# semicolonTransistor/rust-ray-tracing

Hardware: AMD Instinct MI355X
Metric: Msamples/s (pixels×spp/s), 1920×1080·512spp·500 spheres; 1/2/4/8 GPU (higher is better)
Workload: dtype f32

## Files before the change

### rust-ray-tracing_amd/csrc/rt_common.hpp

```cpp
#pragma once
#include <hip/hip_runtime.h>
#include <stdint.h>
#include <stdio.h>
#include <stdlib.h>
#include <string.h>
#include <algorithm>
#include <array>
#include <initializer_list>
#include <chrono>
#include <cmath>
#include <limits>
#include <mutex>
#include <string>
#include <type_traits>
#include <vector>

#include "../../include/rt_mi355x.h"
#include "rt_device.hpp"
#include "rt_formats.hpp"
#include "rt_experiments.hpp"

namespace rt {

template <typename T> struct alignas(64) SphGroup { T v[64 / sizeof(T)]; };

template <typename T>
__device__ __forceinline__ SphGroup<T> load_group(const __attribute__((address_space(4))) T* f, uint32_t g) {
    constexpr int NE = 64 / sizeof(T);
    SphGroup<T> r;
#pragma unroll
    for (int e = 0; e < NE; ++e) r.v[e] = f[g * NE + e];
    return r;
}

typedef float f2 __attribute__((ext_vector_type(2)));
struct Q4 { uint32_t x, y, z, w; };

struct alignas(32) BoxGroup { float v[kBoxFloats]; };
__device__ __forceinline__ BoxGroup load_box(const __attribute__((address_space(4))) float* f, uint32_t g) {
    BoxGroup r;
#pragma unroll
    for (uint32_t e = 0; e < kBoxFloats; ++e) r.v[e] = f[g * kBoxFloats + e];
    return r;
}
__device__ __forceinline__ f2 fma2(f2 a, f2 b, f2 c) { return __builtin_elementwise_fma(a, b, c); }

template <typename T> struct KParams {
    const T* sph;
    const T* cen;
    uint32_t n_groups;
    const MatT<T>* mats;
    uint32_t n_spheres;
    uint32_t W, H;
    double rW, rH;
    T center[3], ulc[3], vu[3], vv[3], du[3], dv[3];
    uint32_t spp, P, C, depth, flags, s_sel, k0, k1;
    uint32_t row_begin, row_step, col_begin, col_count;
    uint8_t* rgb;
    double* lin;
    unsigned long long* segs;
    uint32_t* err;
    uint32_t* counter;
    uint32_t blk_g;
    uint32_t n_items;
    char* scratch;
    size_t scratch_stride;
    uint32_t vbytes, sbytes;
    uint32_t swide;
    const T* camsph;
    const float* fsph;
    const float* camf;
    uint32_t n_fgroups;
    float f_cmax, f_r2max;
    float f_r2min;
    float f_ir2, f_hir2, f_isr;
    const float* cull;
    const float* cullc;
    uint32_t n_clp, n_supc;
    const T* camx;
    const T* rsph;
    const float* rfsph;
    const float* ftop;
    const float* fsup;
    const float* fmeg;
    uint32_t n_mg;
    const float* lfsph;
    const float* lclb;
    const float* lsup;
    const float* lmeg;
    const float* lgig;
    uint32_t n_gg;
    float l_r2max, l_hir2, l_isr;
    const uint64_t* mtiers;
    float mt_lo[3], mt_inv;
    uint32_t mt_n[3];
    const uint32_t* ridx;
    uint32_t n_top, n_xg, n_xs;
};

template <typename T> struct SParams {
    KParams<T> k;
    char* rec;
    uint32_t S, nsub;
    uint32_t n_pix;
};

template <typename T> struct WParams {
    SParams<T> s;
    uint32_t s_begin, s_base;
    uint32_t P_cap;
};

struct MapItem { uint32_t pixel, first, end, pad; };
template <typename T> struct IParams {
    WParams<T> w;
    const MapItem* items;
};
template <typename T> struct LParams {
    WParams<T> w;
    const uint32_t* list;
};

constexpr int kSegShards = 256;
constexpr uint32_t kFlagPinholeInternal = 0x80000000u;
constexpr int kWavesF32 = 6;
constexpr int kWavesF64 = 4;
constexpr int kWavesMegaF32 = 6;
constexpr uint64_t kW6PixelsPerWave = 24;
template <typename T> constexpr int kWavesModes = sizeof(T) == 4 ? 6 : 4;
constexpr int kSegStride = 32;

enum WorkCounter : uint32_t {
    kWBox = 0,
    kWFilt = 1,
    kWExact = 2,
    kWCone = 3,
    kWCExact = 4,
    kNWork = 5,
};
constexpr int kWorkSlot = 11;
constexpr int kDirectSkySlot = 16;
static_assert(kWorkSlot + kNWork <= kDirectSkySlot && kDirectSkySlot < kSegStride, "counters past the shard's slots");
__shared__ unsigned long long g_work[4][kNWork];
__device__ __forceinline__ void work_add(uint32_t i, uint32_t n) {
    const uint32_t first = (uint32_t)__builtin_ctzll(__builtin_amdgcn_read_exec());
    if ((threadIdx.x & 63u) == first) atomicAdd(&g_work[threadIdx.x >> 6][i], (unsigned long long)n);
}


__device__ __forceinline__ uint32_t lanes_below(unsigned long long m) {
    return __builtin_amdgcn_mbcnt_hi((uint32_t)(m >> 32), __builtin_amdgcn_mbcnt_lo((uint32_t)m, 0u));
}

template <typename T> using cptr = const __attribute__((address_space(4))) T*;

template <typename T> __device__ __forceinline__ cptr<KParams<T>> cold_args() {
    cptr<KParams<T>> k = (cptr<KParams<T>>)__builtin_amdgcn_kernarg_segment_ptr();
    asm volatile("" : "+s"(k));
    return k;
}
template <typename T> __device__ __forceinline__ cptr<SParams<T>> cold_split_args() {
    cptr<SParams<T>> k = (cptr<SParams<T>>)__builtin_amdgcn_kernarg_segment_ptr();
    asm volatile("" : "+s"(k));
    return k;
}
template <typename T> __device__ __forceinline__ cptr<WParams<T>> cold_window_args() {
    cptr<WParams<T>> k = (cptr<WParams<T>>)__builtin_amdgcn_kernarg_segment_ptr();
    asm volatile("" : "+s"(k));
    return k;
}
template <typename T> __device__ __forceinline__ cptr<IParams<T>> cold_items_args() {
    cptr<IParams<T>> k = (cptr<IParams<T>>)__builtin_amdgcn_kernarg_segment_ptr();
    asm volatile("" : "+s"(k));
    return k;
}
// ... 90 lines not shown
```

### rust-ray-tracing_amd/csrc/rt_experiments.hpp

```cpp
#pragma once

#if defined(RT_PRODUCT) && defined(RT_EXPERIMENT)
#error "RT_PRODUCT and RT_EXPERIMENT are exclusive"
#endif
#if defined(RT_PRODUCT) && (defined(RT_EXP_BLOCK_SAMPLES) || defined(RT_EXP_TMUL) || defined(RT_EXP_LMAP_CAP) ||      \
                            defined(RT_EXP_DUP_FINISH) || defined(RT_EXP_DUP_CAMRAY) || defined(RT_EXP_DUP_CAM) ||     \
                            defined(RT_EXP_DUP_SCATTER) || defined(RT_EXP_DUP_SWEEP) || defined(RT_EXP_DUP_CLBOX) ||   \
                            defined(RT_EXP_DUP_FILTER) || defined(RT_EXP_DUP_SUPBOX) || defined(RT_EXP_DUP_MEGABOX) || \
                            defined(RT_EXP_DUP_PLIST) || defined(RT_EXP_DUP_REPLAY) || defined(RT_EXP_DUP_REDUCE) ||   \
                            defined(RT_EXP_TIMELINE) || \
                            defined(RT_KSTATS))
#error "an experiment macro in the product build"
#endif
#ifndef RT_SRC_HASH
#define RT_SRC_HASH "unknown"
#endif
#ifdef RT_EXPERIMENT
#define RT_BUILD_KIND "experiment"
#else
#define RT_BUILD_KIND "product"
#endif

namespace rt {

#ifdef RT_EXP_BLOCK_SAMPLES
constexpr uint32_t kBlockSamples = RT_EXP_BLOCK_SAMPLES;
#else
constexpr uint32_t kBlockSamples = 32768;
#endif
#ifdef RT_EXP_TMUL
constexpr uint32_t kTMul = RT_EXP_TMUL;
#else
constexpr uint32_t kTMul = 8;
#endif
#ifdef RT_EXP_LMAP_CAP
constexpr uint32_t kLMapCap = RT_EXP_LMAP_CAP;
#else
constexpr uint32_t kLMapCap = 512;
#endif

#ifdef RT_KSTATS
__shared__ unsigned long long g_kst[4][8];
__device__ __forceinline__ void kstat(uint32_t i, uint32_t n = 1) {
    const unsigned long long ex = __builtin_amdgcn_read_exec();
    if ((threadIdx.x & 63u) == (uint32_t)__builtin_ctzll(ex)) atomicAdd(&g_kst[threadIdx.x >> 6][i], (unsigned long long)n);
}
#define KSTAT(...) kstat(__VA_ARGS__)
#else
#define KSTAT(...) ((void)0)
#endif

}
```

### rust-ray-tracing_amd/csrc/rt_kernel.hip

```cpp
#include "rt_trace.hpp"
#include "rt_layout.hpp"
#include "rt_split_plan.hpp"
#include "rt_progressive_plan.hpp"

#include <chrono>
#include <mutex>
#include <string>

using namespace rt;

static thread_local std::string g_err;
static int fail(int code, const std::string& msg) {
    g_err = msg;
    return code;
}
#define HIPCHK(x)                                                                     \
    do {                                                                              \
        hipError_t e_ = (x);                                                          \
        if (e_ != hipSuccess) return fail(RT_ERR_HIP, std::string(#x ": ") + hipGetErrorString(e_)); \
    } while (0)

struct DeviceBuffer {
    void* p = nullptr;
    size_t bytes = 0;
// ... 51 lines not shown
    PinnedStage& operator=(const PinnedStage&) = delete;
    PinnedStage& operator=(PinnedStage&& o) noexcept {
        if (this != &o) {
            reset();
            p = o.p; bytes = o.bytes; ev = o.ev; pending = o.pending;
            o.p = nullptr; o.bytes = 0; o.ev = nullptr; o.pending = false;
        }
        return *this;
    }
    ~PinnedStage() { reset(); }
    void reset() {
        if (pending) (void)hipEventSynchronize(ev);
        if (ev) (void)hipEventDestroy(ev);
        if (p) (void)hipHostFree(p);
        p = nullptr; bytes = 0; ev = nullptr; pending = false;
    }
};
static int stage_reserve(PinnedStage& g, size_t n) {
    if (!g.ev) HIPCHK(hipEventCreateWithFlags(&g.ev, hipEventDisableTiming));
    if (g.pending) {
        HIPCHK(hipEventSynchronize(g.ev));
        g.pending = false;
    }
    if (n <= g.bytes) return RT_OK;
    if (g.p) HIPCHK(hipHostFree(g.p));
    g.p = nullptr;
    g.bytes = 0;
    HIPCHK(hipHostMalloc(&g.p, n, hipHostMallocDefault));
    g.bytes = n;
    return RT_OK;
}

template <typename T> struct DeviceScene {
    DeviceBuffer sph, cen, fsph, rsph, rfsph, top, sup, meg, lfs, lbx[4], clus, mats;
    DeviceBuffer cam, camf, camx, cull, cullc;
    TableConsts k;
    struct CamKey { bool valid = false; double center[3] = {0, 0, 0}; uint32_t scalar = 0, off = 0; } camkey;
    void reset() { *this = DeviceScene(); }
};
template <typename T> static int upload_scene(DeviceScene<T>& d, const SceneTables<T>& t) {
    int rc = RT_OK;
    auto up = [&](DeviceBuffer& dst, const auto& v) { if (rc == RT_OK) rc = upload(dst, v); };
    auto room = [&](DeviceBuffer& dst, size_t bytes) { if (rc == RT_OK) rc = reserve(dst, bytes); };
    up(d.sph, t.sph); up(d.cen, t.cen); up(d.fsph, t.fsph);
    up(d.rsph, t.rsph); up(d.rfsph, t.rfsph);
    up(d.top, t.top); up(d.sup, t.sup); up(d.meg, t.meg);
    up(d.lfs, t.lfs);
    for (int lv = 0; lv < 4; ++lv) up(d.lbx[lv], t.lbx[lv]);
    up(d.clus, t.clus); up(d.mats, t.mats);
    room(d.cam, t.cam_bytes.cam); room(d.camf, t.cam_bytes.camf); room(d.camx, t.cam_bytes.camx);
    room(d.cull, t.cam_bytes.cull); room(d.cullc, t.cam_bytes.cullc);
    d.k = t.k;
    return rc;
}

struct CountClass {
    uint32_t spp, first, n;
};

struct rt_context {
    int device = 0;
    hipStream_t stream = nullptr;
    hipEvent_t ev_first = nullptr, ev_last = nullptr;
    bool have_first = false;
    DeviceScene<float> d32;
    DeviceScene<double> d64;
    DeviceBuffer ridx, mtiers;
    SceneCounts n;
    template <typename T> DeviceScene<T>& scene() {
        if constexpr (sizeof(T) == 8) return d64; else return d32;
    }
    DeviceBuffer segs, err;
    DeviceBuffer counter;
    DeviceBuffer scratch;
    DeviceBuffer records;
    int n_cu = 0;
    uint64_t samples = 0, pixels = 0;
    hipStream_t last_stream = nullptr;
    bool have_last = false;
// ... 203 lines not shown
    constexpr int W = kWavesSplit<T>;
    return mega ? trace_paths_items<T, W, CAMQ, true> : trace_paths_items<T, W, CAMQ, false>;
}
constexpr uint64_t kScratchBudget = 24ull << 30;

struct FrameArgs {
    const rt_camera* cam;
    uint32_t depth, spp;
    uint64_t seed;
    uint32_t flags;
    rt_tile_range rg;
    void* rgb;
    void* lin;
};
struct SessionWindow {
    char* rec;
    uint32_t cap, s_begin, s_base, S, nsub;
    bool trace, finish;
};

template <typename T>
static void scene_params(rt_context* c, KParams<T>& p) {
    const DeviceScene<T>& d = c->scene<T>();
    const SceneCounts& n = c->n;
    p.sph = (const T*)d.sph.p;
    p.cen = (const T*)d.cen.p;
    p.n_groups = d.k.n_groups;
    p.fsph = (const float*)d.fsph.p;
    p.n_fgroups = n.n_fgroups;
    p.rsph = (const T*)d.rsph.p;
    p.rfsph = (const float*)d.rfsph.p;
    p.ftop = (const float*)d.top.p;
    p.fsup = (const float*)d.sup.p;
    p.fmeg = (const float*)d.meg.p;
    p.n_mg = n.n_mg;
    p.lfsph = (const float*)d.lfs.p;
    p.lclb = (const float*)d.lbx[0].p;
    p.lsup = (const float*)d.lbx[1].p;
    p.lmeg = (const float*)d.lbx[2].p;
    p.lgig = (const float*)d.lbx[3].p;
    p.n_gg = n.n_gg;
    p.mtiers = (const uint64_t*)c->mtiers.p;
    for (int a = 0; a < 3; ++a) { p.mt_lo[a] = n.mt_lo[a]; p.mt_n[a] = n.mt_n[a]; }
    p.mt_inv = n.mt_inv;
    p.l_r2max = d.k.l_r2max;
    p.l_hir2 = d.k.l_hir2;
    p.l_isr = d.k.l_isr;
    p.ridx = (const uint32_t*)c->ridx.p;
    p.n_top = n.n_top;
    p.n_xg = n.n_xg;
    p.n_xs = n.n_xs;
    p.f_cmax = d.k.f_cmax;
    p.f_r2max = d.k.f_r2max;
    p.f_r2min = d.k.f_r2min;
    p.f_ir2 = d.k.f_ir2;
    p.f_hir2 = d.k.f_hir2;
    p.f_isr = d.k.f_isr;
    p.mats = (const MatT<T>*)d.mats.p;
    p.n_spheres = n.n_spheres;
    p.segs = (unsigned long long*)c->segs.p;
    p.err = (uint32_t*)c->err.p;
    p.counter = (uint32_t*)c->counter.p;
}

template <typename T>
static void frame_params(const FrameArgs& a, KParams<T>& p) {
    const rt_camera* cam = a.cam;
// ... 878 lines not shown
                                       uint32_t* items, uint64_t items_capacity) {
    const int rc = progressive_map_plan(n_pixels, done, target, resident_waves, samples_per_item, n_items, items,
                                        items_capacity);
    if (rc != kPlanOk)
        return fail(rc, "rt_progressive_map_plan: a NULL array or output, no pixels, a target below done, too small an "
                        "item capacity (invalid); a target above 2^20, more than 0x7FFFFFFF pixels or items (unsupported)");
    return RT_OK;
}

extern "C" int rt_progressive_end(rt_context* c) {
    if (!c) return fail(RT_ERR_INVALID, "rt_progressive_end: NULL context");
    rt_context::Session& s = c->prog;
    if (!s.open) return fail(RT_ERR_INVALID, "rt_progressive_end: no session open on this context");
    HIPCHK(hipSetDevice(c->device));
    if (s.have_stream) HIPCHK(hipStreamSynchronize(s.stream));
    HIPCHK(hipFree(s.rec));
    s = rt_context::Session{};
    return RT_OK;
}

extern "C" int rt_context_collect(rt_context* c, void* stream, rt_stats* out) {
    if (!c) return fail(RT_ERR_INVALID, "rt_context_collect: NULL context");
    HIPCHK(hipSetDevice(c->device));
    hipStream_t st = (hipStream_t)stream;
    HIPCHK(hipStreamSynchronize(st));
    std::vector<unsigned long long> segs(kSegShards * kSegStride);
    uint32_t err = 0;
    HIPCHK(hipMemcpy(segs.data(), c->segs.p, segs.size() * sizeof(unsigned long long), hipMemcpyDeviceToHost));
    HIPCHK(hipMemcpy(&err, c->err.p, sizeof(uint32_t), hipMemcpyDeviceToHost));
    float ms = 0.f;
    if (c->have_first) HIPCHK(hipEventElapsedTime(&ms, c->ev_first, c->ev_last));
    HIPCHK(hipMemset(c->segs.p, 0, segs.size() * sizeof(unsigned long long)));
    HIPCHK(hipMemset(c->err.p, 0, 16));
    uint64_t total = 0, slots = 0, iters = 0, dsky = 0, kst[8] = {0, 0, 0, 0, 0, 0, 0, 0}, work[kNWork] = {};
    for (int i = 0; i < kSegShards; ++i)
        for (int j = 0; j < 8; ++j) kst[j] += segs[(size_t)i * kSegStride + 3 + j];
    if (kst[0] | kst[1] | kst[2] | kst[3])
        fprintf(stderr, "rt_kstats: general taken_groups %llu sweeps %llu clusters %llu top_groups %llu  camera "
                "candidates %llu sweeps %llu  finish_pixel %llu  filter_lanes_passing %llu\n",
                (unsigned long long)kst[0], (unsigned long long)kst[1], (unsigned long long)kst[4],
                (unsigned long long)kst[5], (unsigned long long)kst[2], (unsigned long long)kst[3],
                (unsigned long long)kst[6], (unsigned long long)kst[7]);
    for (int i = 0; i < kSegShards; ++i) {
        total += segs[(size_t)i * kSegStride];
        slots += segs[(size_t)i * kSegStride + 1];
        iters += segs[(size_t)i * kSegStride + 2];
        dsky += segs[(size_t)i * kSegStride + kDirectSkySlot];
        for (uint32_t j = 0; j < kNWork; ++j) work[j] += segs[(size_t)i * kSegStride + kWorkSlot + j];
    }
    if (out) {
        memset(out, 0, sizeof(*out));
        out->kernel_ms = ms;
        out->pixels = c->pixels;
        out->samples = c->samples;
        out->ray_segments = total;
        out->lane_slots = slots;
        out->bounce_iters = iters;
        out->pixels_per_second = ms > 0.f ? (double)c->pixels / ((double)ms * 1e-3) : 0.0;
        out->box_groups = work[kWBox];
        out->filter_groups = work[kWFilt];
        out->exact_tests = work[kWExact];
        out->cone_tests = work[kWCone];
        out->camera_exact_tests = work[kWCExact];
        out->direct_sky_samples = dsky;
        out->kernel_id = c->last_kernel_id;
        out->kernel_wg_per_cu = c->last_wg_per_cu;
    }
    c->have_first = false;
    c->pixels = c->samples = 0;
    c->last_kernel_id = c->last_wg_per_cu = 0;
    if (err) return fail(RT_ERR_RANGE, "a pixel channel exceeded 2.0 (Color::to_u8_array would panic, color.rs:55-57)");
    return RT_OK;
}

extern "C" int rt_device_alloc(rt_context* c, size_t bytes, void** out) {
// ... 48 lines not shown
```

### rust-ray-tracing_amd/csrc/rt_layout.hpp

```cpp
#pragma once
#include <stdint.h>
#include <string.h>
#include <algorithm>
#include <array>
#include <cmath>
#include <limits>
#include <vector>

#include "../../include/rt_mi355x.h"
#include "rt_formats.hpp"

using namespace rt;

static inline float round_up_f32(double v) {
    float f = (float)v;
    if ((double)f < v) f = std::nextafter(f, std::numeric_limits<float>::infinity());
    return f;
}

template <typename T>
static void pack_scene(const rt_scene* s, std::vector<T>& grp, std::vector<T>& cen, std::vector<MatT<T>>& mats,
                       uint32_t& n_groups) {
    const uint32_t G = kGroup<T>;
    const uint32_t n = s->n_spheres;
// ... 529 lines not shown
                const double dx = (double)cen[4 * i] - C[0], dy = (double)cen[4 * i + 1] - C[1],
                             dz = (double)cen[4 * i + 2] - C[2];
                R = std::max(R, std::sqrt(dx * dx + dy * dy + dz * dz) + std::fabs((double)cen[4 * i + 3]));
            }
        out[4 * at] = C[0]; out[4 * at + 1] = C[1]; out[4 * at + 2] = C[2];
        out[4 * at + 3] = std::isfinite(R) ? R * (1.0 + 0x1.0p-40) : INFINITY;
    };
    for (uint32_t k = 0; k < ncl; ++k) sphere(k, k, 1);
    if (n_supc)
        for (uint32_t k = 0; k < nsup; ++k) sphere(n_clp + k, 4 * k, 4);
}

static std::vector<float> inline_stream(const std::vector<float>& src, size_t n_xg, const std::vector<float>* rg32,
                                        const std::vector<uint32_t>& ridx, const std::vector<float>* frame) {
    const size_t blk = 96, ngf = src.size() / 16 - 1, nxg = n_xg, nk = (ngf - nxg) / 4;
    std::vector<float> rx((size_t)16 * nxg + blk * nk + 32, 0.0f);
    for (size_t g = 0; g < 16 * nxg; ++g) rx[g] = src[g];
    for (size_t k = 0; k < nk; ++k) {
        float* b = &rx[16 * nxg + blk * k];
        for (size_t j = 0; j < 64; ++j) b[j] = src[16 * (nxg + 4 * k) + j];
        for (size_t q = 0; q < 4; ++q) {
            const size_t g = nxg + 4 * k + q;
            uint32_t rec[8] = {0u, 0u, 0u, 0u, 0u, 0u, 0u, 0u};
            if (rg32) for (int h = 0; h < 4; ++h) memcpy(&rec[h], &(*rg32)[16 * g + 8 * (h / 2) + 6 + (h % 2)], 4);
            for (int j = 0; j < 4; ++j) rec[4 + j] = 4 * g + j < ridx.size() ? ridx[4 * g + j] : 0xFFFFFFFFu;
            memcpy(b + 64 + 8 * q, rec, 32);
        }
        if (frame) for (size_t j = 0; j < 4; ++j) { b[64 + j] = (*frame)[8 * k + j]; b[72 + j] = (*frame)[8 * k + 4 + j]; }
    }
    for (size_t j = 0; j < 16; ++j) rx[16 * nxg + blk * nk + j] = src[16 * ngf + j];
    return rx;
}

struct TableConsts {
    uint32_t n_groups = 0;
    float f_cmax = 0, f_r2max = 0, f_r2min = 0;
    float f_ir2 = 0, f_hir2 = 0, f_isr = 0;
    float l_r2max = 0, l_r2min = 0;
    float l_hir2 = 0, l_isr = 0;
};
struct CamTableBytes { size_t cam = 0, camf = 0, camx = 0, cull = 0, cullc = 0; };

template <typename T> struct SceneTables {
    std::vector<T> sph, cen;
    std::vector<float> fsph;
    std::vector<T> rsph;
    std::vector<float> rfsph;
    std::vector<float> top, sup, meg;
    std::vector<float> lfs;
    std::vector<float> lbx[4];
    std::vector<double> clus;
    std::vector<MatT<T>> mats;
    TableConsts k;
    CamTableBytes cam_bytes;
};
struct SceneCounts {
    uint32_t n_spheres = 0;
    uint32_t n_fgroups = 0;
    uint32_t n_top = 0, n_xg = 0, n_xs = 0;
    uint32_t n_mg = 0, n_gg = 0;
    uint32_t n_cslots = 0, n_clp = 0;
    uint32_t n_supc = 0;
    uint32_t n_cull = 0;
    float mt_lo[3] = {0, 0, 0}, mt_inv = 0;
    uint32_t mt_n[3] = {1, 1, 1};
};
struct SceneImage {
    SceneTables<double> t64;
    SceneTables<float> t32;
    std::vector<uint32_t> ridx;
    std::vector<uint64_t> mtiers;
    SceneCounts n;
    template <typename T> const SceneTables<T>& tables() const {
        if constexpr (sizeof(T) == 8) return t64; else return t32;
    }
};

template <typename T>
static void build_tables(const rt_scene* s, const SweepLayout& L, const SceneImage& im, SceneTables<T>& t,
                         uint32_t& n_fgroups, std::vector<float>* wme) {
    std::vector<MatT<T>> mats;
    std::vector<float> frec, rf;
    pack_scene(s, t.sph, t.cen, mats, t.k.n_groups);
    pack_filter(t.cen, s->n_spheres, t.fsph, n_fgroups, t.k.f_cmax, t.k.f_r2max, t.k.f_r2min, frec);
    pack_sweep(t.cen, frec, L, t.rsph, rf, t.top, t.k.f_cmax, t.k.f_r2max, t.sup, t.meg);
    const std::vector<float>* rg32 = nullptr;
    if constexpr (sizeof(T) == 4) rg32 = &t.rsph;
    t.rfsph = inline_stream(rf, L.n_xg, rg32, im.ridx, nullptr);
    if (!t.meg.empty()) {
        std::vector<float> lf, lr, q;
        pack_local(t.cen, L, t.top, lf, lr, q);
        pack_local_boxes(t.cen, L, q, t.lbx[0], t.lbx[1], t.lbx[2], t.lbx[3], t.k.l_r2max, t.k.l_r2min, wme);
        t.lfs = inline_stream(lf, L.n_xg, nullptr, im.ridx, &lr);
    }
    cluster_bounds(t.cen, L, im.n.n_clp, im.n.n_supc, t.clus);
    t.mats.resize(s->n_spheres ? s->n_spheres : 1);
    for (size_t i = 0; i < t.mats.size(); ++i) {
        const uint32_t m = i < s->n_spheres ? s->material[i] : 0u;
        if (m < mats.size()) t.mats[i] = mats[m];
    }
    TableConsts& k = t.k;
    const double r2m = (double)k.f_r2min;
    k.f_ir2 = round_up_f32(1.0 / r2m);
    k.f_hir2 = round_up_f32(0.5 / r2m);
    k.f_isr = round_up_f32(8.0 * 0x1.0p-24 / std::sqrt(r2m));
    const double l2m = (double)k.l_r2min;
    k.l_hir2 = round_up_f32((double)kFilterMargin * 0.5 / l2m);
    k.l_isr = round_up_f32(8.0 * 0x1.0p-24 / std::sqrt(l2m));
    t.cam_bytes.cam = t.sph.size() * sizeof(T);
    t.cam_bytes.camf = t.fsph.size() * sizeof(float);
    t.cam_bytes.camx = (size_t)4 * im.n.n_cslots * sizeof(T);
    t.cam_bytes.cull = (size_t)4 * im.n.n_cslots * sizeof(float);
    t.cam_bytes.cullc = t.clus.size() / 4 * 4 * sizeof(float);
}

static SceneImage build_scene_image(const rt_scene* s) {
    SceneImage im;
    const SweepLayout L = build_layout(s);
    const uint32_t ncl = (uint32_t)L.members.size();
    im.n.n_spheres = s->n_spheres;
    im.n.n_top = ncl / 4;
// ... 23 lines not shown
```

### rust-ray-tracing_amd/csrc/rt_sweep.hpp

```cpp
#pragma once
#include "rt_common.hpp"

namespace rt {

__device__ __forceinline__ void filter_group(const SphGroup<float>& cur, f2 K0, f2 K1, f2 K2, f2 K3, f2& r0, f2& r1) {
    const f2 cx0 = {cur.v[0], cur.v[1]}, cy0 = {cur.v[2], cur.v[3]}, cz0 = {cur.v[4], cur.v[5]}, rr0 = {cur.v[6], cur.v[7]};
    const f2 cx1 = {cur.v[8], cur.v[9]}, cy1 = {cur.v[10], cur.v[11]}, cz1 = {cur.v[12], cur.v[13]}, rr1 = {cur.v[14], cur.v[15]};
    f2 a0, b0, a1, b1;
    asm volatile(
        "v_pk_fma_f32 %[a0], %[cz0], %[K0], %[K3] op_sel:[0,1,0] op_sel_hi:[1,1,0]\n\t"
        "v_pk_fma_f32 %[b0], %[cz0], %[K2], %[K3] op_sel:[0,0,1] op_sel_hi:[1,0,1]\n\t"
        "v_pk_fma_f32 %[a1], %[cz1], %[K0], %[K3] op_sel:[0,1,0] op_sel_hi:[1,1,0]\n\t"
        "v_pk_fma_f32 %[b1], %[cz1], %[K2], %[K3] op_sel:[0,0,1] op_sel_hi:[1,0,1]\n\t"
        "v_pk_fma_f32 %[a0], %[cx0], %[K0], %[a0] op_sel_hi:[1,0,1]\n\t"
        "v_pk_fma_f32 %[b0], %[cy0], %[K1], %[b0] op_sel:[0,1,0] op_sel_hi:[1,1,1]\n\t"
        "v_pk_fma_f32 %[a1], %[cx1], %[K0], %[a1] op_sel_hi:[1,0,1]\n\t"
        "v_pk_fma_f32 %[b1], %[cy1], %[K1], %[b1] op_sel:[0,1,0] op_sel_hi:[1,1,1]\n\t"
        "v_pk_fma_f32 %[b0], %[cx0], %[K1], %[b0] op_sel_hi:[1,0,1]\n\t"
        "v_pk_fma_f32 %[b1], %[cx1], %[K1], %[b1] op_sel_hi:[1,0,1]\n\t"
        "v_pk_fma_f32 %[r0], %[b0], %[b0], %[rr0] neg_lo:[1,0,0] neg_hi:[1,0,0]\n\t"
        "v_pk_fma_f32 %[r1], %[b1], %[b1], %[rr1] neg_lo:[1,0,0] neg_hi:[1,0,0]\n\t"
        "v_pk_fma_f32 %[r0], %[a0], %[a0], %[r0] neg_lo:[1,0,0] neg_hi:[1,0,0]\n\t"
        "v_pk_fma_f32 %[r1], %[a1], %[a1], %[r1] neg_lo:[1,0,0] neg_hi:[1,0,0]"
        : [a0] "=&v"(a0), [b0] "=&v"(b0), [a1] "=&v"(a1), [b1] "=&v"(b1), [r0] "=&v"(r0), [r1] "=&v"(r1)
// ... 319 lines not shown
                        hb = fma2(ocz, dz, fma2(ocy, dy, ocx * dx));
                        const f2 c = fma2(ocz, ocz, fma2(ocy, ocy, ocx * ocx)) - r2;
                        disc = fma2(hb, hb, na * c);
                    }
                    if (cand_f(hb.x, disc.x)) hit(hb.x, disc.x, q ? si.z : si.x);
                    if (cand_f(hb.y, disc.y)) hit(hb.y, disc.y, q ? si.w : si.y);
                }
            } else {
                const SphGroup<T> c0 = load_group(fe, 2 * g), c1 = load_group(fe, 2 * g + 1);
                T hb[4], disc[4];
#pragma unroll
                for (uint32_t j = 0; j < 4; ++j) {
                    if (!((pairs >> j) & 1u)) continue;
                    const T* v = j < 2 ? &c0.v[4 * j] : &c1.v[4 * (j - 2)];
                    const V3<T> oc = mk(o.x - v[0], o.y - v[1], o.z - v[2]);
                    if constexpr (SCALAR) {
                        hb[j] = dot(oc, d);
                        disc[j] = hb[j] * hb[j] - a * (len2(oc) - v[3]);
                    } else {
                        hb[j] = pk_dot(oc, d);
                        const T c = pk_len2(oc) - v[3];
                        disc[j] = fma(hb[j], hb[j], -a * c);
                    }
                }
                const Q4 si = sidx(g, ip);
                const uint32_t sv[4] = {si.x, si.y, si.z, si.w};
#pragma unroll
                for (uint32_t j = 0; j < 4; ++j)
                    if (((pairs >> j) & 1u) && cand_f(hb[j], disc[j])) hit(hb[j], disc[j], sv[j]);
            }
        };
        const uint32_t nxg = qa.n_xg, ntop = qa.n_top;
        uint32_t n_box = 0, n_filt = 0, n_exact = 0;
        auto flush = [&](cptr<float> blk, uint32_t cand) {
            if constexpr (sizeof(T) == 4) {
                while (__ballot(cand != 0u) != 0ull) {
                    KSTAT(0);
                    ++n_exact;
                    if (cand != 0u) {
                        const uint32_t b = (uint32_t)__builtin_ctz(cand);
                        cand &= cand - 1u;
                        const uint32_t s = (b & 15u) ^ 15u;
                        const uint32_t cb = (b & 16u) * 6u;
                        const uint32_t ic = cb + (((s & 14u) << 2) | (s & 1u));
                        const uint32_t ir = cb + (((s & 12u) << 1) | (s & 3u));
                        const float cx = blk[ic], cy = blk[ic + 2u], cz = blk[ic + 4u], r2 = blk[64u + ir];
                        uint32_t si = ((cptr<uint32_t>)blk)[68u + ir];
                        const float ocx = o.x - cx, ocy = o.y - cy, ocz = o.z - cz;
                        float hb, disc;
                        if constexpr (SCALAR) {
                            hb = (ocx * d.x + ocy * d.y) + ocz * d.z;
                            const float c = ((ocx * ocx + ocy * ocy) + ocz * ocz) - r2;
                            disc = hb * hb - a * c;
                        } else {
                            hb = __builtin_fmaf(ocz, d.z, __builtin_fmaf(ocy, d.y, ocx * d.x));
                            const float c = __builtin_fmaf(ocz, ocz, __builtin_fmaf(ocy, ocy, ocx * ocx)) - r2;
                            disc = __builtin_fmaf(hb, hb, -a * c);
                        }
                        asm volatile("" : "+v"(si));
                        if (cand_f(hb, disc)) hit(hb, disc, si);
                    }
                }
            }
        };
        for (uint32_t g = 0; g < nxg; ++g) {
            const uint32_t pr = sizeof(T) == 4 ? (4u * g + 2u >= qa.n_xs ? 1u : 3u) : 15u;
            n_exact += pr == 1u ? 2u : 4u;
            exact4(g, pr);
        }
        cptr<float> ft = (cptr<float>)__builtin_assume_aligned(qa.ftop, 32);
        cptr<float> fs = (cptr<float>)__builtin_assume_aligned(qa.fsup, 32);
        const uint32_t nsg = (ntop + 3u) / 4u;
        auto walk_super = [&](uint32_t sup) {
            KSTAT(5);
            ++n_box;
            uint32_t mask;
            if constexpr (MEGA) {
                mask = lmask(load_lbox((cptr<float>)__builtin_assume_aligned(qa.lclb, 64), sup));
            }
            else mask = box_mask(load_box(ft, sup), B0, B1, B2, B3, B4, btf());
            uint32_t c01 = 0u, c23 = 0u;
            while (mask != 0u) {
                const uint32_t kj = (uint32_t)__builtin_ctz(mask);
                const uint32_t kc = 4u * sup + kj;
                const uint32_t g0 = nxg + 4u * kc;
                mask &= mask - 1u;
                KSTAT(4);
                n_filt += 4u;
                f2 L0 = K0, L1 = K1, L2 = K2, L3 = K3;
                cptr<float> fg = ff;
                if constexpr (MEGA) {
                    const auto& ql = *cold_args<T>();
                    fg = (cptr<float>)__builtin_assume_aligned(ql.lfsph, 64) + 16u * nxg + 96u * kc;
                    const f2 Ckxy = {fg[64], fg[65]};
                    const float Ckz = fg[66];
                    const float Rc = fg[67], r2x = fg[72], ir2 = fg[73];
                    f2 opxy;
                    float opz;
                    if constexpr (sizeof(T) == 4) {
                        opxy = f2{o.x, o.y} - Ckxy;
                        opz = o.z - Ckz;
                    } else {
                        opxy = f2{(float)(o.x - (double)Ckxy.x), (float)(o.y - (double)Ckxy.y)};
                        opz = (float)(o.z - (double)Ckz);
                    }
                    const float opx = opxy.x, opy = opxy.y;
                    const float pmk = ((fabsf(opx) + fabsf(opy)) + fabsf(opz)) + Rc;
                    const float mk = kFilterMargin * __builtin_fmaf(pmk, pmk, r2x);
                    const float sgk = __builtin_amdgcn_rsqf(__builtin_fmaf(mk, ir2, 1.0f));
                    L0 = K0 * sgk; L1 = K1 * sgk; L2 = K2 * sgk;
                    const float oe1l = __builtin_fmaf(opz, L0.y, opx * L0.x);
                    const float oe2l = __builtin_fmaf(opz, L2.x, __builtin_fmaf(opy, L1.y, opx * L1.x));
                    L3 = f2{-oe1l, -oe2l};
                }
                constexpr bool kInl = sizeof(T) == 4 && !MEGA && !CAMT;
                const cptr<float> fgb = MEGA ? fg : ff + 16u * nxg + 96u * kc;
                uint32_t fm = 0xFFFFu;
                sphere_loop(fgb, 4u, [&](const SphGroup<float>& cur, uint32_t g) {
                    f2 Dv[2];
                    filter_group(cur, L0, L1, L2, L3, Dv[0], Dv[1]);
                    if constexpr (kInl) {
                        fm = __builtin_amdgcn_alignbit(fm, __float_as_uint(Dv[0].x), 31u);
                        fm = __builtin_amdgcn_alignbit(fm, __float_as_uint(Dv[0].y), 31u);
                        fm = __builtin_amdgcn_alignbit(fm, __float_as_uint(Dv[1].x), 31u);
                        fm = __builtin_amdgcn_alignbit(fm, __float_as_uint(Dv[1].y), 31u);
                        return;
                    }
                    const uint32_t s0 = __float_as_uint(Dv[0].x) & __float_as_uint(Dv[0].y);
                    const uint32_t s1 = __float_as_uint(Dv[1].x) & __float_as_uint(Dv[1].y);
                    const unsigned long long fpass = __ballot(is_cand(~(s0 & s1)));
                    KSTAT(7, (uint32_t)__popcll(fpass));
                    if (fpass != 0ull) {
                        uint32_t pairs;
                        if constexpr (sizeof(T) == 4) {
                            pairs = (__ballot(!is_cand(s0)) != 0ull ? 1u : 0u) | (__ballot(!is_cand(s1)) != 0ull ? 2u : 0u);
                            n_exact += 2u * (uint32_t)__builtin_popcount(pairs);
                        } else {
                            auto ps = [](float D) -> bool { return (int32_t)__float_as_uint(D) >= 0; };
                            pairs = (__ballot(ps(Dv[0].x)) != 0ull ? 1u : 0u) | (__ballot(ps(Dv[0].y)) != 0ull ? 2u : 0u) |
                                    (__ballot(ps(Dv[1].x)) != 0ull ? 4u : 0u) | (__ballot(ps(Dv[1].y)) != 0ull ? 8u : 0u);
                            n_exact += (uint32_t)__builtin_popcount(pairs);
                        }
                        exact4(g0 + g, pairs, fgb + 68u + 8u * g);
                    }
                });
                if constexpr (kInl) {
                    if (kj < 2u) c01 |= ~fm << (16u * kj);
                    else c23 |= ~fm << (16u * kj - 32u);
                }
            }
            if constexpr (sizeof(T) == 4 && !MEGA) {
                KSTAT(7, (uint32_t)__popcll(__ballot((c01 | c23) != 0u)));
                const cptr<float> sb = ff + 16u * nxg + 384u * sup;
                flush(sb, c01);
                flush(sb + 192u, c23);
            }
        };
        if constexpr (MEGA) {
            cptr<float> lm = (cptr<float>)__builtin_assume_aligned(qa.lmeg, 64);
            cptr<float> ls = (cptr<float>)__builtin_assume_aligned(qa.lsup, 64);
            const uint32_t ntg = qa.n_mg;
            auto walk_mega = [&](uint32_t nd) {
                ++n_box;
                uint32_t smask = lmask(load_lbox(ls, nd));
                if (4u * nd + 4u > ntop) smask &= (1u << (ntop - 4u * nd)) - 1u;
                while (smask != 0u) {
                    const uint32_t sup = 4u * nd + (uint32_t)__builtin_ctz(smask);
                    smask &= smask - 1u;
                    walk_super(sup);
                }
            };
            const uint32_t span = ntg <= 16u ? 16u : 8u;
            constexpr uint32_t kTest = 1;
            for (uint32_t t0 = 0; t0 < ntg; t0 += span) {
                const uint32_t nt = min(span, ntg - t0);
                const uint64_t valid = 4u * (t0 + nt) > nsg ? (1ull << (nsg - 4u * t0)) - 1ull : ~0ull;
                uint64_t T0 = 0, T1 = 0;
                if (span == 16u) {
                    const auto& qt = *cold_args<T>();
                    auto cell = [](float v, float lo, float inv, uint32_t n) -> uint32_t {
                        const float c = fminf(fmaxf((v - lo) * inv, 0.0f), (float)(n - 1u));
                        return __builtin_amdgcn_readfirstlane((uint32_t)c);
                    };
                    const uint32_t cx = cell((float)o.x, qt.mt_lo[0], qt.mt_inv, qt.mt_n[0]);
                    const uint32_t cy = cell((float)o.y, qt.mt_lo[1], qt.mt_inv, qt.mt_n[1]);
                    const uint32_t cz = cell((float)o.z, qt.mt_lo[2], qt.mt_inv, qt.mt_n[2]);
                    const uint32_t ci = 4u * (cx + qt.mt_n[0] * (cy + qt.mt_n[1] * cz));
                    cptr<uint64_t> tt = (cptr<uint64_t>)__builtin_assume_aligned(qt.mtiers, 32);
                    T0 = tt[ci] & valid;
// ... 20 lines not shown
                            n_box += nt;
                            for (uint32_t t1 = 0; t1 < nt; t1 += 8u)
                                lbox_loop(lm + 32u * (t0 + t1), min(8u, nt - t1), [&](const LBoxGroup& cur, uint32_t t) {
                                    KSTAT(5);
                                    tm |= (uint64_t)lmask(cur) << (4u * (t1 + t));
                                });
                        }
                        tm &= valid;
                    }
                    uint64_t w = k == 0u ? (kTest == 0u ? tm & T0 : T0)
                                         : (k == 1u ? (kTest <= 1u ? tm & T1 : T1) & ~T0 : tm & ~T1);
                    while (w != 0ull) {
                        const uint32_t nd = 4u * t0 + (uint32_t)__builtin_ctzll(w);
                        w &= w - 1ull;
                        walk_mega(nd);
                    }
                }
            }
        } else {
            for (uint32_t t0 = 0; t0 < nsg; t0 += 8u) {
                uint32_t tmask = 0;
                n_box += min(8u, nsg - t0);
                box_loop(fs + kBoxFloats * t0, min(8u, nsg - t0), [&](const BoxGroup& cur, uint32_t t) {
                    KSTAT(5);
                    tmask |= box_mask(cur, B0, B1, B2, B3, B4, btf()) << (4u * t);
                });
                while (tmask != 0u) {
                    const uint32_t nd = 4u * t0 + (uint32_t)__builtin_ctz(tmask);
                    tmask &= tmask - 1u;
                    if (nd >= ntop) break;
                    walk_super(nd);
                }
            }
        }
        work_add(kWBox, n_box);
        work_add(kWFilt, n_filt);
        work_add(kWExact, n_exact);
    }
    t_out = bh.bt();
    return bh.bi();
}

}
```

### rust-ray-tracing_amd/csrc/rt_trace_body.hpp

```cpp
    constexpr bool SC = MODE == kModeScalar;
    static_assert(!SPLIT || (MODE == kModeV2 && !ROOT2), "the sample-parallel kernels cover the live path only");
    static_assert(!ITEMS || (SPLIT && !WIN), "an item table replaces the window's decode");
    constexpr bool kF64Park = sizeof(T) == 8 && W >= 5;
    constexpr uint32_t QW = CAMQ ? 4 : 1, QN = CAMQ ? (kF64Park ? 64u : kQCap) : 1;
    __shared__ unsigned long long wcount[4][4];
    __shared__ __attribute__((aligned(16))) uint32_t s_hist[4][64];
    __shared__ __attribute__((aligned(16))) T s_stage[4][3][64];
    using IS = std::conditional_t<SPLIT, IssueStateS, IssueState>;
    __shared__ IS s_is[4];
    __shared__ unsigned long long s_pool;
    __shared__ uint32_t s_dry;
    __shared__ uint32_t q_sid[QW][QN];
    __shared__ uint32_t s_slotpix[4][kSlots];
    __shared__ uint32_t s_item[4][kSlots];
    __shared__ int q_hit[QW][QN];
    __shared__ T q_t[QW][QN], q_d[QW][3][QN];
    __shared__ alignas(16) uint16_t s_clist[QW][CAMQ ? kSlots : 1][kCList];
    constexpr bool kPark = (sizeof(T) == 4 && W >= 6) || kF64Park;
    constexpr bool kParkC = kPark && (MEGA || (sizeof(T) == 4 && W == 6));
    __shared__ T s_park[kPark ? 4 : 1][kParkC ? 9 : 6][64];
    constexpr bool kLMap = MODE == kModeV2 && !MEGA && kLMapCap > 0u && sizeof(T) == 8 && !kF64Park;
    __shared__ __attribute__((aligned(16))) uint16_t s_lmap[kLMap ? 4 : 1][kLMap ? kLMapCap : 2];
    const uint32_t lane = threadIdx.x & 63u;
    const uint32_t wave = __builtin_amdgcn_readfirstlane(threadIdx.x >> 6);
    if (lane == 0) { wcount[wave][0] = 0; wcount[wave][1] = 0; wcount[wave][2] = 0; wcount[wave][3] = 0; }
    if (lane < kNWork) g_work[wave][lane] = 0ull;
#ifdef RT_KSTATS
    if (lane < 8) g_kst[wave][lane] = 0;
#endif
    if constexpr (SPLIT) {
        if (lane == 0) s_is[wave] = IssueStateS{};
    } else {
        if (lane == 0) s_is[wave] = IssueState{0u, 0u, cold_args<T>()->spp, 0u, 0u, 0u, 0u, 0u, 0u, 0u, 0u, 0u};
    }
    {
        const auto& q = *cold_args<T>();
        uint32_t b0 = 0, b1 = 0;
        const bool got = guided_block(q.n_items, max(1u, kTMul * gridDim.x), q.blk_g, blockIdx.x, b0, b1);
        if (threadIdx.x == 0) {
            s_pool = got ? ((unsigned long long)b0 << 32) | b1 : 0ull;
            s_dry = 0u;
        }
    }
    __syncthreads();
    V3<T> o = mk(T(0), T(0), T(0)), d = o, c = o;
    uint32_t ss = 0, k = 0;
    constexpr bool kParkSS = MEGA;
    uint32_t* const ssp = (uint32_t*)&s_stage[wave][0][0] + lane;
    auto ss_get = [&]() -> uint32_t {
        if constexpr (kParkSS) { asm volatile("" ::: "memory"); return *ssp; }
        else return ss;
    };
    auto ss_set = [&](uint32_t v) {
        if constexpr (kParkSS) *ssp = v;
        else ss = v;
    };
    if constexpr (kParkSS) *ssp = 0u;
    constexpr uint32_t kSlotNZ = 0x80000000u;
    uint32_t slot_left = 0;
    auto sid_of = [](uint32_t v) -> uint32_t { return v & 0x1FFFFFFFu; };
    auto slot_of = [](uint32_t v) -> uint32_t { return v >> 29; };
// ... 323 lines not shown
        } else if (scat) {
            k += 1u;
        }
        if (__ballot(live) == 0ull) break;
        const uint32_t depth = cold_args<T>()->depth;
        const bool act = live && k < depth;
        hit_i = -1;
        if (act) hit_i = nearest_hit<T, ROOT2, SC, false, MEGA>(p, o, d, hit_t);
        const unsigned long long bact = __ballot(act);
        if (lane == 0 && bact) { wcount[wave][0] += (uint32_t)__popcll(bact); wcount[wave][1] += 64u; }
        const bool skyhit = act && hit_i < 0;
        const bool term = live && (!act || skyhit || k + 1 == depth);
        scat = act && hit_i >= 0 && k + 1 < depth;
        if constexpr (kPark) {
            if (MODE != kModeV2) { V3<T> po, pd; unpark(po, pd); d = pd; }
        }
        if constexpr (kParkC) c = unpark_c();
        {
            const uint32_t ssv = ss_get();
            terminate(term, skyhit, skyhit ? k : depth, slot_of(ssv), sid_of(ssv), c, d);
        }
        live = live && !term;
    }
    if (lane == 0) {
        const auto& q = *cold_args<T>();
        const uint32_t gw = blockIdx.x * (blockDim.x >> 6) + wave;
        unsigned long long* cc = &q.segs[(gw & (kSegShards - 1)) * kSegStride];
        atomicAdd(cc + 0, wcount[wave][0]);
        atomicAdd(cc + 1, wcount[wave][1]);
        atomicAdd(cc + 2, wcount[wave][2]);
        if (wcount[wave][3]) atomicAdd(cc + kDirectSkySlot, wcount[wave][3]);
        for (uint32_t i = 0; i < kNWork; ++i) atomicAdd(cc + kWorkSlot + i, g_work[wave][i]);
#ifdef RT_KSTATS
        for (int i = 0; i < 8; ++i) atomicAdd(cc + 3 + i, g_kst[wave][i]);
#endif
    }
```

Baseline: 39140.

## Flush exact sphere tests per child pair from a flat float4 record table

Adds a host-packed flat table (rflat) of one float4 per sphere slot (center xyz, radius squared) and a parallel index table. The exact-test flush now reads one aligned 16-byte record plus an index instead of decoding a swizzled interleaved block with scattered scalar loads. It also flushes after each pair of child boxes is finished rather than once per super group, which shrinks the candidate mask and the divergent loop length but adds more ballot-driven flush calls. Kstats counters are extended to measure flush behaviour, and the unused meg buffer upload is dropped.

```diff
diff --git a/rust-ray-tracing_amd/csrc/rt_common.hpp b/rust-ray-tracing_amd/csrc/rt_common.hpp
--- a/rust-ray-tracing_amd/csrc/rt_common.hpp
+++ b/rust-ray-tracing_amd/csrc/rt_common.hpp
@@ -34,6 +34,7 @@
 }
 
 typedef float f2 __attribute__((ext_vector_type(2)));
+typedef float F4 __attribute__((ext_vector_type(4)));
 struct Q4 { uint32_t x, y, z, w; };
 
 struct alignas(32) BoxGroup { float v[kBoxFloats]; };
@@ -82,7 +83,7 @@
     const float* rfsph;
     const float* ftop;
     const float* fsup;
-    const float* fmeg;
+    const float* rflat;
     uint32_t n_mg;
     const float* lfsph;
     const float* lclb;
@@ -141,6 +142,8 @@
 constexpr int kWorkSlot = 11;
 constexpr int kDirectSkySlot = 16;
 static_assert(kWorkSlot + kNWork <= kDirectSkySlot && kDirectSkySlot < kSegStride, "counters past the shard's slots");
+static_assert(kKstatSlot >= 3 && kKstatSlot + kNKstat1 <= kWorkSlot && kKstatSlot2 > kDirectSkySlot &&
+              kKstatSlot2 + (kNKstat - kNKstat1) <= kSegStride, "kstats counters over another counter's slot");
 __shared__ unsigned long long g_work[4][kNWork];
 __device__ __forceinline__ void work_add(uint32_t i, uint32_t n) {
     const uint32_t first = (uint32_t)__builtin_ctzll(__builtin_amdgcn_read_exec());
diff --git a/rust-ray-tracing_amd/csrc/rt_experiments.hpp b/rust-ray-tracing_amd/csrc/rt_experiments.hpp
--- a/rust-ray-tracing_amd/csrc/rt_experiments.hpp
+++ b/rust-ray-tracing_amd/csrc/rt_experiments.hpp
@@ -8,6 +8,7 @@
                             defined(RT_EXP_DUP_SCATTER) || defined(RT_EXP_DUP_SWEEP) || defined(RT_EXP_DUP_CLBOX) ||   \
                             defined(RT_EXP_DUP_FILTER) || defined(RT_EXP_DUP_SUPBOX) || defined(RT_EXP_DUP_MEGABOX) || \
                             defined(RT_EXP_DUP_PLIST) || defined(RT_EXP_DUP_REPLAY) || defined(RT_EXP_DUP_REDUCE) ||   \
+                            defined(RT_EXP_DUP_FLUSH) ||                                                                \
                             defined(RT_EXP_TIMELINE) || \
                             defined(RT_KSTATS))
 #error "an experiment macro in the product build"
@@ -39,8 +40,10 @@
 constexpr uint32_t kLMapCap = 512;
 #endif
 
+constexpr int kNKstat = 13, kNKstat1 = 8, kKstatSlot = 3, kKstatSlot2 = 17;
+constexpr int kstat_slot(int i) { return i < kNKstat1 ? kKstatSlot + i : kKstatSlot2 + (i - kNKstat1); }
 #ifdef RT_KSTATS
-__shared__ unsigned long long g_kst[4][8];
+__shared__ unsigned long long g_kst[4][kNKstat];
 __device__ __forceinline__ void kstat(uint32_t i, uint32_t n = 1) {
     const unsigned long long ex = __builtin_amdgcn_read_exec();
     if ((threadIdx.x & 63u) == (uint32_t)__builtin_ctzll(ex)) atomicAdd(&g_kst[threadIdx.x >> 6][i], (unsigned long long)n);
diff --git a/rust-ray-tracing_amd/csrc/rt_kernel.hip b/rust-ray-tracing_amd/csrc/rt_kernel.hip
--- a/rust-ray-tracing_amd/csrc/rt_kernel.hip
+++ b/rust-ray-tracing_amd/csrc/rt_kernel.hip
@@ -107,7 +107,7 @@
 }
 
 template <typename T> struct DeviceScene {
-    DeviceBuffer sph, cen, fsph, rsph, rfsph, top, sup, meg, lfs, lbx[4], clus, mats;
+    DeviceBuffer sph, cen, fsph, rsph, rfsph, rflat, top, sup, lfs, lbx[4], clus, mats;
     DeviceBuffer cam, camf, camx, cull, cullc;
     TableConsts k;
     struct CamKey { bool valid = false; double center[3] = {0, 0, 0}; uint32_t scalar = 0, off = 0; } camkey;
@@ -118,8 +118,8 @@
     auto up = [&](DeviceBuffer& dst, const auto& v) { if (rc == RT_OK) rc = upload(dst, v); };
     auto room = [&](DeviceBuffer& dst, size_t bytes) { if (rc == RT_OK) rc = reserve(dst, bytes); };
     up(d.sph, t.sph); up(d.cen, t.cen); up(d.fsph, t.fsph);
-    up(d.rsph, t.rsph); up(d.rfsph, t.rfsph);
-    up(d.top, t.top); up(d.sup, t.sup); up(d.meg, t.meg);
+    up(d.rsph, t.rsph); up(d.rfsph, t.rfsph); up(d.rflat, t.rflat);
+    up(d.top, t.top); up(d.sup, t.sup);
     up(d.lfs, t.lfs);
     for (int lv = 0; lv < 4; ++lv) up(d.lbx[lv], t.lbx[lv]);
     up(d.clus, t.clus); up(d.mats, t.mats);
@@ -389,7 +389,7 @@
     p.rfsph = (const float*)d.rfsph.p;
     p.ftop = (const float*)d.top.p;
     p.fsup = (const float*)d.sup.p;
-    p.fmeg = (const float*)d.meg.p;
+    p.rflat = (const float*)d.rflat.p;
     p.n_mg = n.n_mg;
     p.lfsph = (const float*)d.lfs.p;
     p.lclb = (const float*)d.lbx[0].p;
@@ -1334,15 +1334,19 @@
     if (c->have_first) HIPCHK(hipEventElapsedTime(&ms, c->ev_first, c->ev_last));
     HIPCHK(hipMemset(c->segs.p, 0, segs.size() * sizeof(unsigned long long)));
     HIPCHK(hipMemset(c->err.p, 0, 16));
-    uint64_t total = 0, slots = 0, iters = 0, dsky = 0, kst[8] = {0, 0, 0, 0, 0, 0, 0, 0}, work[kNWork] = {};
+    uint64_t total = 0, slots = 0, iters = 0, dsky = 0, kst[kNKstat] = {}, work[kNWork] = {};
     for (int i = 0; i < kSegShards; ++i)
-        for (int j = 0; j < 8; ++j) kst[j] += segs[(size_t)i * kSegStride + 3 + j];
-    if (kst[0] | kst[1] | kst[2] | kst[3])
+        for (int j = 0; j < kNKstat; ++j) kst[j] += segs[(size_t)i * kSegStride + kstat_slot(j)];
+    if (kst[0] | kst[1] | kst[2] | kst[3]) {
         fprintf(stderr, "rt_kstats: general taken_groups %llu sweeps %llu clusters %llu top_groups %llu  camera "
                 "candidates %llu sweeps %llu  finish_pixel %llu  filter_lanes_passing %llu\n",
                 (unsigned long long)kst[0], (unsigned long long)kst[1], (unsigned long long)kst[4],
                 (unsigned long long)kst[5], (unsigned long long)kst[2], (unsigned long long)kst[3],
                 (unsigned long long)kst[6], (unsigned long long)kst[7]);
+        fprintf(stderr, "rt_kstats: flush steps_per_super_max %llu steps_per_sweep_max %llu lanes_two_supers %llu "
+                "lanes_any %llu lanes_two_pairs %llu\n", (unsigned long long)kst[8], (unsigned long long)kst[9],
+                (unsigned long long)kst[10], (unsigned long long)kst[11], (unsigned long long)kst[12]);
+    }
     for (int i = 0; i < kSegShards; ++i) {
         total += segs[(size_t)i * kSegStride];
         slots += segs[(size_t)i * kSegStride + 1];
diff --git a/rust-ray-tracing_amd/csrc/rt_layout.hpp b/rust-ray-tracing_amd/csrc/rt_layout.hpp
--- a/rust-ray-tracing_amd/csrc/rt_layout.hpp
+++ b/rust-ray-tracing_amd/csrc/rt_layout.hpp
@@ -585,6 +585,15 @@
     return rx;
 }
 
+static std::vector<float> pack_flat(const std::vector<float>& rg32, size_t n_slots) {
+    std::vector<float> fl((size_t)4 * n_slots, 0.0f);
+    const size_t ns = (rg32.size() / 16 - 1) * 4;
+    for (size_t i = 0; i < n_slots; ++i)
+        for (int f = 0; f < 4; ++f)
+            fl[4 * i + f] = i < ns ? rg32[16 * (i / 4) + 8 * ((i % 4) / 2) + 2 * f + (i % 2)] : (f == 3 ? -INFINITY : 0.0f);
+    return fl;
+}
+
 struct TableConsts {
     uint32_t n_groups = 0;
     float f_cmax = 0, f_r2max = 0, f_r2min = 0;
@@ -599,7 +608,9 @@
     std::vector<float> fsph;
     std::vector<T> rsph;
     std::vector<float> rfsph;
-    std::vector<float> top, sup, meg;
+    std::vector<float> rflat;
+    std::vector<float> top, sup;
+    std::vector<float> meg;
     std::vector<float> lfs;
     std::vector<float> lbx[4];
     std::vector<double> clus;
@@ -640,6 +651,7 @@
     const std::vector<float>* rg32 = nullptr;
     if constexpr (sizeof(T) == 4) rg32 = &t.rsph;
     t.rfsph = inline_stream(rf, L.n_xg, rg32, im.ridx, nullptr);
+    if constexpr (sizeof(T) == 4) t.rflat = pack_flat(t.rsph, im.ridx.size());
     if (!t.meg.empty()) {
         std::vector<float> lf, lr, q;
         pack_local(t.cen, L, t.top, lf, lr, q);
diff --git a/rust-ray-tracing_amd/csrc/rt_sweep.hpp b/rust-ray-tracing_amd/csrc/rt_sweep.hpp
--- a/rust-ray-tracing_amd/csrc/rt_sweep.hpp
+++ b/rust-ray-tracing_amd/csrc/rt_sweep.hpp
@@ -375,29 +375,28 @@
         };
         const uint32_t nxg = qa.n_xg, ntop = qa.n_top;
         uint32_t n_box = 0, n_filt = 0, n_exact = 0;
-        auto flush = [&](cptr<float> blk, uint32_t cand) {
+        auto flush = [&](uint32_t ofs, uint32_t cand) {
             if constexpr (sizeof(T) == 4) {
+                const cptr<char> fl = (cptr<char>)__builtin_assume_aligned(qa.rflat, 16) + 64u * nxg;
+                const cptr<char> ri = (cptr<char>)__builtin_assume_aligned(qa.ridx, 16) + 16u * nxg;
                 while (__ballot(cand != 0u) != 0ull) {
                     KSTAT(0);
                     ++n_exact;
                     if (cand != 0u) {
                         const uint32_t b = (uint32_t)__builtin_ctz(cand);
                         cand &= cand - 1u;
-                        const uint32_t s = (b & 15u) ^ 15u;
-                        const uint32_t cb = (b & 16u) * 6u;
-                        const uint32_t ic = cb + (((s & 14u) << 2) | (s & 1u));
-                        const uint32_t ir = cb + (((s & 12u) << 1) | (s & 3u));
-                        const float cx = blk[ic], cy = blk[ic + 2u], cz = blk[ic + 4u], r2 = blk[64u + ir];
-                        uint32_t si = ((cptr<uint32_t>)blk)[68u + ir];
-                        const float ocx = o.x - cx, ocy = o.y - cy, ocz = o.z - cz;
+                        const uint32_t at = ofs + ((b ^ 15u) << 4);
+                        const F4 rec = *(cptr<F4>)(fl + at);
+                        uint32_t si = *(cptr<uint32_t>)(ri + (at >> 2));
+                        const float ocx = o.x - rec.x, ocy = o.y - rec.y, ocz = o.z - rec.z;
                         float hb, disc;
                         if constexpr (SCALAR) {
                             hb = (ocx * d.x + ocy * d.y) + ocz * d.z;
-                            const float c = ((ocx * ocx + ocy * ocy) + ocz * ocz) - r2;
+                            const float c = ((ocx * ocx + ocy * ocy) + ocz * ocz) - rec.w;
                             disc = hb * hb - a * c;
                         } else {
                             hb = __builtin_fmaf(ocz, d.z, __builtin_fmaf(ocy, d.y, ocx * d.x));
-                            const float c = __builtin_fmaf(ocz, ocz, __builtin_fmaf(ocy, ocy, ocx * ocx)) - r2;
+                            const float c = __builtin_fmaf(ocz, ocz, __builtin_fmaf(ocy, ocy, ocx * ocx)) - rec.w;
                             disc = __builtin_fmaf(hb, hb, -a * c);
                         }
                         asm volatile("" : "+v"(si));
@@ -406,6 +405,15 @@
                 }
             }
         };
+#ifdef RT_KSTATS
+        constexpr bool kInlK = sizeof(T) == 4 && !MEGA && !CAMT;
+        uint32_t ks_cur = 0u, ks_tot = 0u, ks_sup = 0u, ks_pair = 0u;
+        auto wave_max = [](uint32_t v) -> uint32_t {
+            uint32_t m = 0u;
+            while (__ballot(v > m) != 0ull) ++m;
+            return m;
+        };
+#endif
         for (uint32_t g = 0; g < nxg; ++g) {
             const uint32_t pr = sizeof(T) == 4 ? (4u * g + 2u >= qa.n_xs ? 1u : 3u) : 15u;
             n_exact += pr == 1u ? 2u : 4u;
@@ -422,7 +430,7 @@
                 mask = lmask(load_lbox((cptr<float>)__builtin_assume_aligned(qa.lclb, 64), sup));
             }
             else mask = box_mask(load_box(ft, sup), B0, B1, B2, B3, B4, btf());
-            uint32_t c01 = 0u, c23 = 0u;
+            uint32_t cpr = 0u;
             while (mask != 0u) {
                 const uint32_t kj = (uint32_t)__builtin_ctz(mask);
                 const uint32_t kc = 4u * sup + kj;
@@ -488,16 +496,26 @@
                     }
                 });
                 if constexpr (kInl) {
-                    if (kj < 2u) c01 |= ~fm << (16u * kj);
-                    else c23 |= ~fm << (16u * kj - 32u);
-                }
-            }
-            if constexpr (sizeof(T) == 4 && !MEGA) {
-                KSTAT(7, (uint32_t)__popcll(__ballot((c01 | c23) != 0u)));
-                const cptr<float> sb = ff + 16u * nxg + 384u * sup;
-                flush(sb, c01);
-                flush(sb + 192u, c23);
-            }
+                    cpr |= ~fm << (16u * (kj & 1u));
+                    if ((mask & (kj < 2u ? 3u : 12u)) == 0u) {
+#ifdef RT_KSTATS
+                        ks_cur += (uint32_t)__builtin_popcount(cpr);
+                        ks_pair += cpr != 0u ? 1u : 0u;
+#endif
+                        flush(1024u * sup + 512u * (kj >> 1), cpr);
+                        cpr = 0u;
+                    }
+                }
+            }
+#ifdef RT_KSTATS
+            if constexpr (kInlK) {
+                KSTAT(7, (uint32_t)__popcll(__ballot(ks_cur != 0u)));
+                KSTAT(8, wave_max(ks_cur));
+                ks_tot += ks_cur;
+                ks_sup += ks_cur != 0u ? 1u : 0u;
+                ks_cur = 0u;
+            }
+#endif
         };
         if constexpr (MEGA) {
             cptr<float> lm = (cptr<float>)__builtin_assume_aligned(qa.lmeg, 64);
@@ -584,6 +602,14 @@
                     walk_super(nd);
                 }
             }
+#ifdef RT_KSTATS
+            if constexpr (kInlK) {
+                KSTAT(9, wave_max(ks_tot));
+                KSTAT(10, (uint32_t)__popcll(__ballot(ks_sup >= 2u)));
+                KSTAT(11, (uint32_t)__popcll(__ballot(ks_sup >= 1u)));
+                KSTAT(12, (uint32_t)__popcll(__ballot(ks_pair >= 2u)));
+            }
+#endif
         }
         work_add(kWBox, n_box);
         work_add(kWFilt, n_filt);
diff --git a/rust-ray-tracing_amd/csrc/rt_trace_body.hpp b/rust-ray-tracing_amd/csrc/rt_trace_body.hpp
--- a/rust-ray-tracing_amd/csrc/rt_trace_body.hpp
+++ b/rust-ray-tracing_amd/csrc/rt_trace_body.hpp
@@ -26,7 +26,7 @@
     if (lane == 0) { wcount[wave][0] = 0; wcount[wave][1] = 0; wcount[wave][2] = 0; wcount[wave][3] = 0; }
     if (lane < kNWork) g_work[wave][lane] = 0ull;
 #ifdef RT_KSTATS
-    if (lane < 8) g_kst[wave][lane] = 0;
+    if (lane < kNKstat) g_kst[wave][lane] = 0;
 #endif
     if constexpr (SPLIT) {
         if (lane == 0) s_is[wave] = IssueStateS{};
@@ -416,6 +416,6 @@
         if (wcount[wave][3]) atomicAdd(cc + kDirectSkySlot, wcount[wave][3]);
         for (uint32_t i = 0; i < kNWork; ++i) atomicAdd(cc + kWorkSlot + i, g_work[wave][i]);
 #ifdef RT_KSTATS
-        for (int i = 0; i < 8; ++i) atomicAdd(cc + 3 + i, g_kst[wave][i]);
+        for (int i = 0; i < kNKstat; ++i) atomicAdd(cc + kstat_slot(i), g_kst[wave][i]);
 #endif
     }
```

New measurement: 39850, median of 6. +1.8%, better.
